# NVIDIA-Merlin/distributed-embeddings

Hardware: AMD Instinct MI355X
Metric: samples/sec (whole node) DLRM-Criteo-1TB bs/gpu=65536 (higher is better)
Workload: dtype bf16; 1 GPU; model=DLRM-Criteo-1TB, global_batch=65536, batch_per_gpu=65536, embedding_dim=128, parallelism=hybrid dp+mp (strategy=memory_balanced) x1

## Files before the change

distributed_embeddings_amd/csrc/bindings.cpp:

```cpp

#include <torch/extension.h>

#include <c10/hip/HIPStream.h>

#include "ops_api.h"

namespace {

#define CHECK_CUDA(x) TORCH_CHECK((x).is_cuda(), #x " must be on GPU")
#define CHECK_CONTIG(x) TORCH_CHECK((x).is_contiguous(), #x " must be contiguous")

inline hipStream_t current_stream() {
  return c10::hip::getCurrentHIPStream().stream();
}

int log2_ceil(int64_t v) {
  int b = 0;
  while ((int64_t(1) << b) < v) ++b;
  return b;
}


bool use_rocprim_sort() {
  static int v = -1;
// ... 479 lines not shown
              "rehash target must not be smaller");
  launch_hash_reinsert(old_keys.data_ptr<int64_t>(),
                       old_values.data_ptr<int64_t>(), old_keys.numel(),
                       new_keys.data_ptr<int64_t>(),
                       new_values.data_ptr<int64_t>(), new_keys.numel(),
                       current_stream());
}

static bool check_adagrad_state(const torch::Tensor& state,
                                const torch::Tensor& weight) {
  CHECK_CUDA(state); CHECK_CONTIG(state);
  const bool rowwise = state.dim() == 1 && state.size(0) == weight.size(0);
  TORCH_CHECK(rowwise || state.sizes() == weight.sizes(),
              "adagrad state shape mismatch: expected [vocab, width] "
              "(element-wise) or [vocab] (row-wise), got ", state.sizes(),
              " for weight ", weight.sizes());
  TORCH_CHECK(state.dtype() == torch::kFloat32, "adagrad state must be fp32");
  return rowwise;
}

static int64_t* sr_ptr(const std::optional<torch::Tensor>& sr,
                       const torch::Tensor& weight) {
  if (!sr.has_value()) return nullptr;
  const torch::Tensor& t = *sr;
  CHECK_CUDA(t); CHECK_CONTIG(t);
  TORCH_CHECK(t.dtype() == torch::kInt64 && t.dim() == 1 && t.numel() == 2,
              "sr must be an int64 [2] tensor {seed, step}");
  TORCH_CHECK(t.device() == weight.device(),
              "sr must be on the weight's device");
  TORCH_CHECK(weight.dtype() == torch::kBFloat16,
              "stochastic rounding needs a bf16 weight: an fp32 weight has "
              "nothing to round");
  return t.data_ptr<int64_t>();
}

static void check_adam_state(const torch::Tensor& state,
                             const torch::Tensor& weight, double beta1,
                             double beta2) {
  CHECK_CUDA(state); CHECK_CONTIG(state);
  TORCH_CHECK(state.dtype() == torch::kFloat32, "adam state must be fp32");
  TORCH_CHECK(state.dim() == 3 && state.size(0) == 2 &&
              state.size(1) == weight.size(0) &&
              state.size(2) == weight.size(1),
              "adam state shape mismatch: expected [2, vocab, width], got ",
              state.sizes(), " for weight ", weight.sizes());
  TORCH_CHECK(state.device() == weight.device(),
              "adam state must be on the weight's device");
  TORCH_CHECK(beta1 >= 0.0 && beta1 < 1.0 && beta2 >= 0.0 && beta2 < 1.0,
              "adam betas must lie in [0, 1), got (", beta1, ", ", beta2, ")");
}

void sparse_row_update(torch::Tensor weight, torch::Tensor state,
                       torch::Tensor ids, torch::Tensor grad, double lr,
                       double eps, bool adagrad,
                       std::optional<torch::Tensor> sr, int64_t adam_step,
                       double beta1, double beta2) {
  CHECK_CUDA(weight); CHECK_CUDA(ids); CHECK_CUDA(grad);
  CHECK_CONTIG(weight); CHECK_CONTIG(ids); CHECK_CONTIG(grad);
  TORCH_CHECK(weight.dtype() == torch::kFloat32 ||
              weight.dtype() == torch::kBFloat16);
  TORCH_CHECK(grad.dtype() == torch::kFloat32);
  TORCH_CHECK(ids.dtype() == torch::kInt64);
  int64_t* sr_p = sr_ptr(sr, weight);
  TORCH_CHECK(adam_step >= 0, "adam_step must not be negative");
  const bool adam = adam_step > 0;
  TORCH_CHECK(!(adam && adagrad), "adam_step and adagrad exclude each other");
  if (adam) check_adam_state(state, weight, beta1, beta2);
  const int64_t n = ids.numel();
  if (n == 0) return;
  float* state_ptr = nullptr;
  bool rowwise = false;
  if (adagrad) {
    rowwise = check_adagrad_state(state, weight);
    state_ptr = state.data_ptr<float>();
  }
  AdamConfig cfg{beta1, beta2, weight.size(0), nullptr, nullptr};
  if (adam) {
    state_ptr = state.data_ptr<float>();
    const double t = (double)adam_step;
    lr = lr * std::sqrt(1.0 - std::pow(beta2, t)) / (1.0 - std::pow(beta1, t));
  }
  launch_sparse_row_update(weight.data_ptr(),
                           weight.dtype() == torch::kBFloat16, state_ptr,
                           ids.data_ptr<int64_t>(), grad.data_ptr<float>(), n,
                           (int)weight.size(1), (float)lr, (float)eps, adagrad,
                           rowwise, sr_p, adam ? &cfg : nullptr,
                           current_stream());
}

void csr_fused_optimizer_apply(torch::Tensor weight, torch::Tensor state,
                               torch::Tensor values, torch::Tensor row_splits,
                               torch::Tensor grad_out, torch::Tensor lr,
                               bool mean, bool adagrad, double eps,
                               std::optional<torch::Tensor> per_id_w,
                               std::optional<torch::Tensor> sr,
                               std::optional<torch::Tensor> adam_step,
                               double beta1, double beta2) {
  CHECK_CUDA(weight); CHECK_CUDA(values); CHECK_CUDA(row_splits);
  CHECK_CUDA(grad_out); CHECK_CUDA(lr);
  CHECK_CONTIG(weight); CHECK_CONTIG(values); CHECK_CONTIG(row_splits);
  CHECK_CONTIG(grad_out);
  TORCH_CHECK(weight.dtype() == torch::kFloat32 ||
              weight.dtype() == torch::kBFloat16);
  TORCH_CHECK((grad_out.dtype() == torch::kFloat32 ||
               grad_out.dtype() == torch::kBFloat16) &&
              lr.dtype() == torch::kFloat32);
  const float* user_w = per_id_w_ptr(per_id_w, values);
  int64_t* sr_p = sr_ptr(sr, weight);
  const bool wbf16 = weight.dtype() == torch::kBFloat16;
  const int64_t num_rows = row_splits.numel() - 1;
  const int64_t nnz = values.numel();
  const int64_t vocab = weight.size(0);
  const int width = (int)weight.size(1);
  const bool adam = adam_step.has_value();
  if (adam) {
    TORCH_CHECK(!adagrad, "adam_step and adagrad exclude each other");
    check_adam_state(state, weight, beta1, beta2);
    const torch::Tensor& t = *adam_step;
    CHECK_CUDA(t); CHECK_CONTIG(t);
    TORCH_CHECK(t.dtype() == torch::kInt64 && t.dim() == 1 && t.numel() == 1,
                "adam_step must be an int64 [1] tensor");
    TORCH_CHECK(t.device() == weight.device(),
                "adam_step must be on the weight's device");
  }
  if (num_rows <= 0 || nnz <= 0) return;
  auto stream = current_stream();
  auto i64 = values.options();
  auto i32 = values.options().dtype(torch::kInt32);
  auto f32 = grad_out.options().dtype(torch::kFloat32);

  auto ss = build_sorted_segments(values, row_splits, vocab, mean, user_w,
                                  stream);
  launch_pad_seg_offsets(ss.seg.data_ptr<int64_t>(), nnz,
                         ss.num_unique.data_ptr<int32_t>(),
                         ss.bounds.data_ptr<int64_t>(), stream);
  auto long_rows = torch::empty({nnz}, i64);
  auto long_count = torch::empty({1}, i32);
  auto work_items = torch::empty({nnz / 64 + 64}, i64);
  auto n_work = torch::empty({1}, i32);
  float* state_ptr = nullptr;
  torch::Tensor scratch;
  float* scratch_ptr = nullptr;
  int64_t scratch_rows = 0;
  bool rowwise = false;
  if (adagrad) {
    rowwise = check_adagrad_state(state, weight);
    state_ptr = state.data_ptr<float>();
  }
  AdamConfig cfg{beta1, beta2, vocab, nullptr, nullptr};
  torch::Tensor a_t;
  if (adam) {
    state_ptr = state.data_ptr<float>();
    a_t = torch::empty({1}, f32);
    cfg.step = adam_step->data_ptr<int64_t>();
    cfg.a_t = a_t.data_ptr<float>();
  }
  if (adagrad || adam || wbf16) {
    scratch_rows = nnz / (128 + 1) + 1;
    scratch = torch::empty({scratch_rows, (int64_t)width}, f32);
    scratch_ptr = scratch.data_ptr<float>();
  }
  launch_sorted_optimizer_update(weight.data_ptr(), wbf16, state_ptr,
                                 (float)eps, ss.sorted_ids.data_ptr<int64_t>(),
                                 ss.seg.data_ptr<int64_t>(),
                                 ss.srow.data_ptr<int64_t>(), ss.sw_ptr(),
                                 grad_out.data_ptr(),
                                 grad_out.dtype() == torch::kBFloat16,
                                 lr.data_ptr<float>(),
                                 ss.num_unique.data_ptr<int32_t>(), nnz, width,
                                 long_rows.data_ptr<int64_t>(),
                                 long_count.data_ptr<int32_t>(),
                                 work_items.data_ptr<int64_t>(),
                                 n_work.data_ptr<int32_t>(), scratch_ptr,
                                 scratch_rows, adagrad, rowwise, sr_p,
                                 adam ? &cfg : nullptr, stream);
}

torch::Tensor stochastic_round_bf16(torch::Tensor x, int64_t seed,
                                    int64_t step, int64_t base_offset) {
  CHECK_CUDA(x); CHECK_CONTIG(x);
  TORCH_CHECK(x.dtype() == torch::kFloat32, "x must be fp32");
  TORCH_CHECK(base_offset >= 0, "base_offset must not be negative");
  auto out = torch::empty(x.sizes(), x.options().dtype(torch::kBFloat16));
  launch_stochastic_round_bf16(x.data_ptr<float>(), out.data_ptr(), x.numel(),
                               seed, step, base_offset, current_stream());
  return out;
}

torch::Tensor dot_interact_fwd(torch::Tensor feats, int64_t out_w) {
  CHECK_CUDA(feats); CHECK_CONTIG(feats);
  TORCH_CHECK(feats.dtype() == torch::kBFloat16, "feats must be bf16");
  TORCH_CHECK(feats.dim() == 3, "feats must be [B, F, D]");
  const int64_t B = feats.size(0);
  const int F = (int)feats.size(1), D = (int)feats.size(2);
  TORCH_CHECK(F <= 32 && D % 32 == 0, "F<=32 and D%32==0 required");
  const int tri_n = F * (F - 1) / 2;
  TORCH_CHECK(out_w >= tri_n + D, "out width too small");
  auto out = torch::empty({B, out_w}, feats.options());
  launch_dot_interact_fwd(feats.data_ptr(), out.data_ptr(), B, F, D,
                          (int)out_w, tri_n, current_stream());
  return out;
}

torch::Tensor dot_interact_fwd_packed(torch::Tensor bottom,
                                      torch::Tensor packed, torch::Tensor perm,
                                      int64_t out_w, bool sample_major) {
  CHECK_CUDA(bottom); CHECK_CUDA(packed); CHECK_CUDA(perm);
  CHECK_CONTIG(bottom); CHECK_CONTIG(packed); CHECK_CONTIG(perm);
  TORCH_CHECK(bottom.dtype() == torch::kBFloat16 &&
              packed.dtype() == torch::kBFloat16, "bf16 required");
  TORCH_CHECK(perm.dtype() == torch::kInt32, "perm must be int32");
  TORCH_CHECK(bottom.dim() == 2 && packed.dim() == 3, "bottom [B,D], packed 3-D");
  const int64_t B = bottom.size(0);
  const int D = (int)bottom.size(1);
  const int P = (int)(sample_major ? packed.size(1) : packed.size(0));
  TORCH_CHECK(packed.size(sample_major ? 0 : 1) == B && packed.size(2) == D,
              "shape mismatch");
  TORCH_CHECK(perm.numel() == P, "perm must have P entries");
  const int F = P + 1;
  TORCH_CHECK(F <= 32 && D % 32 == 0, "F<=32 and D%32==0 required");
  const int tri_n = F * (F - 1) / 2;
  TORCH_CHECK(out_w >= tri_n + D, "out width too small");
  const int64_t sb = sample_major ? P : 1;
  const int64_t sp = sample_major ? 1 : B;
  auto out = torch::empty({B, out_w}, bottom.options());
  launch_dot_interact_fwd_packed(bottom.data_ptr(), packed.data_ptr(),
                                 perm.data_ptr<int>(), out.data_ptr(), B, F, D,
                                 (int)out_w, tri_n, sb, sp, current_stream());
  return out;
}

std::vector<torch::Tensor> dot_interact_bwd_packed(torch::Tensor gout,
                                                   torch::Tensor bottom,
                                                   torch::Tensor packed,
                                                   torch::Tensor perm,
                                                   bool sample_major) {
  CHECK_CUDA(gout); CHECK_CUDA(bottom); CHECK_CUDA(packed); CHECK_CUDA(perm);
  CHECK_CONTIG(gout); CHECK_CONTIG(bottom); CHECK_CONTIG(packed);
  CHECK_CONTIG(perm);
  TORCH_CHECK(gout.dtype() == torch::kBFloat16 &&
              bottom.dtype() == torch::kBFloat16 &&
              packed.dtype() == torch::kBFloat16, "bf16 required");
  TORCH_CHECK(perm.dtype() == torch::kInt32, "perm must be int32");
  const int64_t B = bottom.size(0);
  const int D = (int)bottom.size(1);
  const int P = (int)(sample_major ? packed.size(1) : packed.size(0));
  TORCH_CHECK(perm.numel() == P, "perm must have P entries");
  TORCH_CHECK(packed.size(sample_major ? 0 : 1) == B && packed.size(2) == D,
              "shape mismatch");
  const int F = P + 1;
  const int tri_n = F * (F - 1) / 2;
  const int64_t sb = sample_major ? P : 1;
  const int64_t sp = sample_major ? 1 : B;
  auto gbottom = torch::empty_like(bottom);
  auto gpacked = torch::empty_like(packed);
  launch_dot_interact_bwd_packed(gout.data_ptr(), bottom.data_ptr(),
                                 packed.data_ptr(), perm.data_ptr<int>(),
                                 gbottom.data_ptr(), gpacked.data_ptr(), B, F,
                                 D, (int)gout.size(1), tri_n, sb, sp,
                                 current_stream());
  return {gbottom, gpacked};
}

torch::Tensor dot_interact_bwd(torch::Tensor gout, torch::Tensor feats) {
  CHECK_CUDA(gout); CHECK_CUDA(feats);
  CHECK_CONTIG(gout); CHECK_CONTIG(feats);
  TORCH_CHECK(gout.dtype() == torch::kBFloat16 &&
              feats.dtype() == torch::kBFloat16);
  const int64_t B = feats.size(0);
  const int F = (int)feats.size(1), D = (int)feats.size(2);
  const int tri_n = F * (F - 1) / 2;
  auto gfeats = torch::empty_like(feats);
  launch_dot_interact_bwd(gout.data_ptr(), feats.data_ptr(),
                          gfeats.data_ptr(), B, F, D, (int)gout.size(1), tri_n,
                          current_stream());
  return gfeats;
}

std::vector<torch::Tensor> relu_bwd_bias_grad(torch::Tensor grad_out,
                                              torch::Tensor y) {
  CHECK_CUDA(grad_out); CHECK_CUDA(y);
  CHECK_CONTIG(grad_out); CHECK_CONTIG(y);
  TORCH_CHECK(grad_out.dtype() == torch::kBFloat16 &&
              y.dtype() == torch::kBFloat16, "bf16 required");
  TORCH_CHECK(grad_out.dim() == 2 && grad_out.sizes() == y.sizes(),
              "grad_out and y must be [B, N]");
  const int64_t B = grad_out.size(0);
  const int64_t N = grad_out.size(1);
  TORCH_CHECK(N % 8 == 0 && N < (int64_t(1) << 31), "N % 8 == 0 required");
  auto grad_in = torch::empty_like(grad_out);
  if (B == 0 || N == 0) {
    return {grad_in, torch::zeros({N}, grad_out.options())};
  }
  auto bias_grad = torch::empty({N}, grad_out.options());
  int64_t rows_per_chunk = 0, num_chunks = 0;
  relu_bwd_bias_grad_plan(B, (int)N, &rows_per_chunk, &num_chunks);
  auto slab = torch::empty({num_chunks, N},
                           grad_out.options().dtype(torch::kFloat32));
  launch_relu_bwd_bias_grad(grad_out.data_ptr(), y.data_ptr(),
                            grad_in.data_ptr(), slab.data_ptr<float>(),
                            bias_grad.data_ptr(), B, (int)N, rows_per_chunk,
                            num_chunks, current_stream());
  return {grad_in, bias_grad};
}

}

PYBIND11_MODULE(TORCH_EXTENSION_NAME, m) {
  m.def("csr_lookup_forward", &csr_lookup_forward,
        "CSR segmented gather-reduce forward (gfx950)",
        pybind11::arg("params"), pybind11::arg("values"),
        pybind11::arg("row_splits"), pybind11::arg("mean"),
        pybind11::arg("out_bf16") = false,
        pybind11::arg("per_id_w") = pybind11::none());
  m.def("csr_lookup_forward_q8", &csr_lookup_forward_q8,
        "CSR gather-reduce from an int8 row-wise quantized table (gfx950)",
        pybind11::arg("packed"), pybind11::arg("values"),
        pybind11::arg("row_splits"), pybind11::arg("mean"),
        pybind11::arg("out_bf16") = false,
        pybind11::arg("per_id_w") = pybind11::none());
  m.def("quantize_rows_q8", &quantize_rows_q8,
        "fp32/bf16 [n, width] -> int8 row-wise packed [n, width + 8] (gfx950)",
        pybind11::arg("weight"));
  m.def("dequantize_rows_q8", &dequantize_rows_q8,
        "int8 row-wise packed [n, width + 8] -> fp32 [n, width] (gfx950)",
        pybind11::arg("packed"));
  m.def("csr_lookup_backward", &csr_lookup_backward,
        "sparse backward: sort + unique + segmented sum (gfx950)",
        pybind11::arg("grad_out"), pybind11::arg("values"),
        pybind11::arg("row_splits"), pybind11::arg("vocab"),
        pybind11::arg("mean"), pybind11::arg("per_id_w") = pybind11::none());
  m.def("csr_lookup_weight_grad", &csr_lookup_weight_grad,
        "gradient of the per-id weights of a weighted lookup (gfx950)",
        pybind11::arg("grad_out"), pybind11::arg("params"),
        pybind11::arg("values"), pybind11::arg("row_splits"),
        pybind11::arg("mean"));
  m.def("debug_sort_ids", &debug_sort_ids,
        "TESTS ONLY: the backward's id sort -> (sorted_ids, sorted_pos)",
        pybind11::arg("values"), pybind11::arg("vocab"),
        pybind11::arg("variant") = -1, pybind11::arg("sort") = "default");
  m.def("debug_sorted_segments", &debug_sorted_segments,
        "TESTS ONLY: the backward's sorted-segment view -> (sorted_ids, "
        "srow, sw or None, seg, unique_ids, num_unique, bounds)",
        pybind11::arg("values"), pybind11::arg("row_splits"),
        pybind11::arg("vocab"), pybind11::arg("mean"),
        pybind11::arg("per_id_w") = pybind11::none(),
        pybind11::arg("padded") = false, pybind11::arg("variant") = -1,
        pybind11::arg("sort") = "default");
  m.def("debug_sort_variant_tiles", &debug_sort_variant_tiles,
        "TESTS ONLY: keys per block of each radix-sort tile variant");
  m.def("row_to_split", &row_to_split, "COO rows -> CSR splits (gfx950)");
  m.def("hash_rehash", &hash_rehash,
        "re-insert occupied (key,value) pairs into a larger hash (gfx950)");
  m.def("integer_lookup", &integer_lookup,
        "open-addressing hash vocab build + lookup (gfx950)");
  m.def("sparse_row_update", &sparse_row_update,
        "fused sparse SGD/Adagrad/row-wise Adagrad/lazy Adam row update "
        "(gfx950)",
        pybind11::arg("weight"), pybind11::arg("state"), pybind11::arg("ids"),
        pybind11::arg("grad"), pybind11::arg("lr"), pybind11::arg("eps"),
        pybind11::arg("adagrad"), pybind11::arg("sr") = pybind11::none(),
        pybind11::arg("adam_step") = 0, pybind11::arg("beta1") = 0.9,
        pybind11::arg("beta2") = 0.999);
  m.def("csr_fused_optimizer_apply", &csr_fused_optimizer_apply,
        "in-backward fused SGD/Adagrad/row-wise Adagrad/lazy Adam update "
        "(gfx950)",
        pybind11::arg("weight"), pybind11::arg("state"),
        pybind11::arg("values"), pybind11::arg("row_splits"),
        pybind11::arg("grad_out"), pybind11::arg("lr"), pybind11::arg("mean"),
        pybind11::arg("adagrad"), pybind11::arg("eps"),
        pybind11::arg("per_id_w") = pybind11::none(),
        pybind11::arg("sr") = pybind11::none(),
        pybind11::arg("adam_step") = pybind11::none(),
        pybind11::arg("beta1") = 0.9, pybind11::arg("beta2") = 0.999);
  m.def("stochastic_round_bf16", &stochastic_round_bf16,
        "fp32 -> bf16 with the fused optimizers' stochastic rounding (gfx950)",
        pybind11::arg("x"), pybind11::arg("seed"), pybind11::arg("step") = 0,
        pybind11::arg("base_offset") = 0);
  m.def("dot_interact_fwd_packed", &dot_interact_fwd_packed,
        "pairwise-dot interaction on (bottom, packed, perm) (MFMA, gfx950)");
  m.def("dot_interact_bwd_packed", &dot_interact_bwd_packed,
        "packed interaction backward -> (gbottom, gpacked) (MFMA, gfx950)");
  m.def("dot_interact_fwd", &dot_interact_fwd,
        "fused DLRM pairwise-dot interaction forward (MFMA bf16, gfx950)");
  m.def("dot_interact_bwd", &dot_interact_bwd,
        "fused DLRM pairwise-dot interaction backward (MFMA bf16, gfx950)");
  m.def("relu_bwd_bias_grad", &relu_bwd_bias_grad,
        "ReLU backward + bias gradient in one pass -> (grad_in, bias_grad) "
        "(gfx950)");
}
```

distributed_embeddings_amd/csrc/ops_api.h:

```cpp
#pragma once

#include <hip/hip_runtime.h>

#include <cstddef>
#include <cstdint>

void launch_csr_lookup_forward(const void* params, bool params_bf16,
                               const int64_t* values, const int64_t* splits,
                               const float* per_id_w, void* out, bool out_bf16,
                               int64_t num_rows, int64_t nnz, int64_t vocab,
                               int width, bool mean, int64_t* long_rows,
                               int32_t* long_count, int64_t* work_items,
                               int32_t* n_work, hipStream_t stream);

void launch_csr_lookup_forward_q8(const void* packed, const int64_t* values,
                                  const int64_t* splits, const float* per_id_w,
                                  void* out, bool out_bf16, int64_t num_rows,
                                  int64_t nnz, int64_t vocab, int width,
                                  bool mean, int64_t* long_rows,
                                  int32_t* long_count, int64_t* work_items,
                                  int32_t* n_work, hipStream_t stream);
void launch_quantize_rows_q8(const void* in, bool in_bf16, void* packed,
                             int64_t n, int width, hipStream_t stream);
void launch_dequantize_rows_q8(const void* packed, float* out, int64_t n,
                               int width, hipStream_t stream);

void launch_row_to_split(const int64_t* rows, int64_t nnz, int64_t num_rows,
                         int64_t* splits, hipStream_t stream);

size_t csr_backward_temp_bytes(int64_t nnz);

void launch_expand_row_ids(const int64_t* splits, int64_t num_rows,
                           int64_t nnz, int32_t* row_ids, float* w, bool mean,
                           const float* user_w, hipStream_t stream);

void launch_csr_weight_grad(const void* params, bool params_bf16,
                            const void* grad_out, bool grad_bf16,
                            const int64_t* values, const int32_t* row_ids,
                            const int64_t* splits, bool mean, float* dw,
                            int64_t nnz, int64_t vocab, int width,
                            hipStream_t stream);

hipError_t run_inclusive_scan_i32(void* temp, size_t temp_bytes,
                                  const int32_t* in, int32_t* out, int64_t n,
                                  hipStream_t stream);

void launch_mark_heads(const int64_t* sorted_ids, int64_t n, int64_t vocab,
                       int32_t* head, hipStream_t stream);

void launch_scatter_unique(const int64_t* sorted_ids, const int32_t* head,
                           const int32_t* pos, int64_t n, int64_t* unique_ids,
                           int64_t* seg_offsets, int32_t* num_unique,
                           hipStream_t stream);

void launch_gather_sorted(const int32_t* perm, const int32_t* row_ids,
                          const float* w, int64_t n, int64_t* srow, float* sw,
                          hipStream_t stream);

void launch_find_valid_bounds(const int64_t* sorted_ids, int64_t n,
                              int64_t vocab, int64_t* valid_end,
                              hipStream_t stream);

void launch_set_seg_end(int64_t* seg_offsets, const int32_t* num_unique,
                        const int64_t* valid_end, hipStream_t stream);

void launch_integer_lookup(const int64_t* keys, int64_t n, int64_t* tkeys,
                           int64_t* tvals, int64_t capacity, int32_t* counts,
                           int64_t max_tokens, void* temp, size_t temp_bytes,
                           int32_t* scratch_flags, int32_t* scratch_pos,
                           int64_t* avail, int32_t* navail, int32_t* next_avail,
                           int64_t* out, hipStream_t stream);

size_t integer_lookup_temp_bytes(int64_t max_tokens);

void launch_hash_reinsert(const int64_t* old_keys, const int64_t* old_vals,
                          int64_t old_cap, int64_t* tkeys, int64_t* tvals,
                          int64_t capacity, hipStream_t stream);

void launch_pad_seg_offsets(int64_t* seg, int64_t n, const int32_t* num_unique,
                            const int64_t* valid_end, hipStream_t stream);

struct AdamConfig {
  double b1, b2;
  int64_t vocab;
  int64_t* step;
  float* a_t;
};

void launch_sorted_optimizer_update(void* weight, bool weight_bf16,
                                    float* state, float eps,
                                    const int64_t* sorted_ids,
                                    const int64_t* seg, const int64_t* srow,
                                    const float* sw, const void* grad_out,
                                    bool grad_bf16,
                                    const float* lr, const int32_t* nu_ptr,
                                    int64_t max_segs, int width,
                                    int64_t* long_rows, int32_t* long_count,
                                    int64_t* work_items, int32_t* n_work,
                                    float* long_scratch, int64_t scratch_rows,
                                    bool adagrad, bool rowwise, int64_t* sr,
                                    const AdamConfig* adam,
                                    hipStream_t stream);

void launch_sparse_row_update(void* weight, bool weight_bf16, float* state,
                              const int64_t* ids, const float* grad,
                              int64_t num_rows, int width, float lr, float eps,
                              bool adagrad, bool rowwise, int64_t* sr,
                              const AdamConfig* adam, hipStream_t stream);

void launch_stochastic_round_bf16(const float* x, void* out, int64_t n,
                                  int64_t seed, int64_t step,
                                  int64_t base_offset, hipStream_t stream);

void launch_dot_interact_fwd_packed(const void* bottom, const void* packed,
                                    const int* perm, void* out, int64_t B,
                                    int F, int D, int out_w, int tri_n,
                                    int64_t sb, int64_t sp,
                                    hipStream_t stream);
void launch_dot_interact_bwd_packed(const void* gout, const void* bottom,
                                    const void* packed, const int* perm,
                                    void* gbottom, void* gpacked, int64_t B,
                                    int F, int D, int out_w, int tri_n,
                                    int64_t sb, int64_t sp,
                                    hipStream_t stream);
void launch_dot_interact_fwd(const void* feats, void* out, int64_t B, int F,
                             int D, int out_w, int tri_n, hipStream_t stream);
void launch_dot_interact_bwd(const void* gout, const void* feats, void* gfeats,
                             int64_t B, int F, int D, int out_w, int tri_n,
                             hipStream_t stream);

void relu_bwd_bias_grad_plan(int64_t B, int N, int64_t* rows_per_chunk,
                             int64_t* num_chunks);
void launch_relu_bwd_bias_grad(const void* grad_out, const void* y,
                               void* grad_in, float* slab, void* bias_grad,
                               int64_t B, int N, int64_t rows_per_chunk,
                               int64_t num_chunks, hipStream_t stream);

size_t custom_radix_sort_hist_elems(int64_t n);
int custom_radix_sort_num_variants();
int custom_radix_sort_variant_tile(int variant);

void custom_radix_sort_keys(const uint64_t* keys_in, uint64_t* keys_out,
                            uint64_t* keys_tmp, int32_t* hist,
                            int32_t* scan_sums, int64_t n, int begin_bit,
                            int end_bit, int variant, hipStream_t stream);

void launch_mask_oob_pack(const int64_t* ids, int64_t n, int64_t vocab,
                          uint64_t* packed, hipStream_t stream);
void launch_unpack_sorted(const uint64_t* packed, int64_t n,
                          int64_t* sorted_ids, int32_t* sorted_pos,
                          hipStream_t stream);
hipError_t run_sort_keys_u64(void* temp, size_t temp_bytes,
                             const uint64_t* keys_in, uint64_t* keys_out,
                             int64_t n, int begin_bit, int end_bit,
                             hipStream_t stream);
size_t rocprim_sort_keys_temp_bytes(int64_t n);
```

distributed_embeddings_amd/ops/mlp.py:

```python

import os
from typing import Tuple

import torch
from torch import nn

from . import _backend


def relu_bwd_bias_grad(grad_out: torch.Tensor,
                       y: torch.Tensor) -> Tuple[torch.Tensor, torch.Tensor]:
    if (grad_out.is_cuda and grad_out.dim() == 2
            and grad_out.dtype == torch.bfloat16 and y.dtype == torch.bfloat16
            and grad_out.shape == y.shape and grad_out.shape[1] % 8 == 0
            and grad_out.is_contiguous() and y.is_contiguous()):
        g, gb = _backend.ops().relu_bwd_bias_grad(grad_out, y)
        return g, gb
    g = torch.ops.aten.threshold_backward(grad_out, y, 0)
    return g, g.sum(0)


class _LinearReLU(torch.autograd.Function):

    @staticmethod
    def forward(ctx, x, w, b):
        xb = x.to(torch.bfloat16)
        wb = w.to(torch.bfloat16)
        y = torch.addmm(b.to(torch.bfloat16), xb, wb.t())
        torch.relu_(y)
        ctx.save_for_backward(xb, wb, y)
        ctx.x_dtype = x.dtype
        return y

    @staticmethod
    @torch.autograd.function.once_differentiable
    def backward(ctx, grad_out):
        xb, wb, y = ctx.saved_tensors
        g, gb = relu_bwd_bias_grad(grad_out, y)
        gx = None
        if ctx.needs_input_grad[0]:
            gx = g.mm(wb).to(ctx.x_dtype)
        gw = g.t().mm(xb)
        return gx, gw, gb


class MLP(nn.Sequential):

    def _fused(self, x: torch.Tensor) -> bool:
        return (x.is_cuda and x.dim() == 2 and torch.is_autocast_enabled()
                and torch.get_autocast_dtype("cuda") == torch.bfloat16
                and os.environ.get("DE_FUSED_MLP", "1") != "0"
                and _backend.available())

    def forward(self, input):
        if not self._fused(input):
            return super().forward(input)
        mods = list(self)
        h = input
        i = 0
        while i < len(mods):
            m = mods[i]
            if (isinstance(m, nn.Linear) and m.bias is not None
                    and m.weight.dtype == torch.float32
                    and m.bias.dtype == torch.float32
                    and i + 1 < len(mods) and isinstance(mods[i + 1], nn.ReLU)
                    and h.dim() == 2):
                h = _LinearReLU.apply(h, m.weight, m.bias)
                i += 2
            else:
                h = m(h)
                i += 1
        return h
```

setup.py:

```python

import os

from setuptools import setup

os.environ.setdefault("PYTORCH_ROCM_ARCH", "gfx950")

from torch.utils.cpp_extension import BuildExtension, CUDAExtension

ext = CUDAExtension(
    name="distributed_embeddings_amd._hip_ops",
    sources=[
        "distributed_embeddings_amd/csrc/bindings.cpp",
        "distributed_embeddings_amd/csrc/embedding_ops.hip",
        "distributed_embeddings_amd/csrc/dot_interact.hip",
        "distributed_embeddings_amd/csrc/radix_sort.hip",
        "distributed_embeddings_amd/csrc/mlp_ops.hip",
    ],
    extra_compile_args={
        "cxx": ["-O3", "-std=c++17"],
        "nvcc": ["-O3", "-std=c++17"],
    },
)

setup(
    name="distributed_embeddings_amd",
    version="0.1.0",
    packages=[
        "distributed_embeddings_amd",
        "distributed_embeddings_amd.ops",
        "distributed_embeddings_amd.layers",
        "distributed_embeddings_amd.parallel",
        "distributed_embeddings_amd.models",
        "distributed_embeddings_amd.utils",
    ],
    ext_modules=[ext],
    cmdclass={"build_ext": BuildExtension},
)
```

Measured before the change: 17.86 million samples/s.

## Add split-K MFMA kernel for MLP weight gradients with tall-skinny shapes

Adds a custom split-K bf16 MFMA GEMM for the linear weight gradient g^T x, where K is the large batch dimension (65536) and M, N are small layer widths. Each workgroup accumulates a K-slice into an fp32 slab, and a second kernel reduces the slices and rounds to bf16. The goal is to fill the GPU on shapes where a standard GEMM yields few output tiles. The cost is an extra fp32 slab write and read, a second launch, and a host-side plan call on every backward.

```diff
diff --git a/distributed_embeddings_amd/csrc/bindings.cpp b/distributed_embeddings_amd/csrc/bindings.cpp
--- a/distributed_embeddings_amd/csrc/bindings.cpp
+++ b/distributed_embeddings_amd/csrc/bindings.cpp
@@ -805,6 +805,40 @@
                             bias_grad.data_ptr(), B, (int)N, rows_per_chunk,
                             num_chunks, current_stream());
   return {grad_in, bias_grad};
+}
+
+torch::Tensor wgrad_splitk(torch::Tensor g, torch::Tensor x, int64_t splitk,
+                           int64_t tile) {
+  CHECK_CUDA(g); CHECK_CUDA(x);
+  CHECK_CONTIG(g); CHECK_CONTIG(x);
+  TORCH_CHECK(g.dtype() == torch::kBFloat16 && x.dtype() == torch::kBFloat16,
+              "bf16 required");
+  TORCH_CHECK(g.dim() == 2 && x.dim() == 2 && g.size(0) == x.size(0),
+              "g must be [K, M] and x [K, N]");
+  const int64_t K = g.size(0), M = g.size(1), N = x.size(1);
+  TORCH_CHECK(splitk >= 0, "splitk must not be negative");
+  TORCH_CHECK(tile >= -1 && tile <= 2, "tile must be -1 (plan), 0, 1 or 2");
+  WgradSplitkPlan plan;
+  TORCH_CHECK(wgrad_splitk_plan_with(K, M, N, splitk, (int)tile, &plan),
+              "wgrad_splitk takes K >= 1, M % 8 == 0 and N % 8 == 0 or "
+              "N <= 16 (tile 2 for N <= 16 only); got K=", K, " M=", M,
+              " N=", N, " tile=", tile);
+  TORCH_CHECK(reinterpret_cast<uintptr_t>(g.data_ptr()) % 16 == 0 &&
+              reinterpret_cast<uintptr_t>(x.data_ptr()) % 16 == 0,
+              "operands must be 16-byte aligned");
+  auto gw = torch::empty({M, N}, g.options());
+  auto slab = torch::empty({plan.splitk, M, plan.np},
+                           g.options().dtype(torch::kFloat32));
+  launch_wgrad_splitk(g.data_ptr(), x.data_ptr(), slab.data_ptr<float>(),
+                      gw.data_ptr(), K, (int)M, (int)N, plan,
+                      current_stream());
+  return gw;
+}
+
+std::vector<int64_t> wgrad_splitk_plan_py(int64_t K, int64_t M, int64_t N) {
+  WgradSplitkPlan plan;
+  if (!wgrad_splitk_plan(K, M, N, &plan)) return {0, 0, -1};
+  return {plan.use ? 1 : 0, plan.splitk, plan.cfg};
 }
 
 }
@@ -891,4 +925,10 @@
   m.def("relu_bwd_bias_grad", &relu_bwd_bias_grad,
         "ReLU backward + bias gradient in one pass -> (grad_in, bias_grad) "
         "(gfx950)");
-}
+  m.def("wgrad_splitk", &wgrad_splitk,
+        "Linear weight gradient bf16(g^T x), split-K (MFMA bf16, gfx950)",
+        pybind11::arg("g"), pybind11::arg("x"), pybind11::arg("splitk") = 0,
+        pybind11::arg("tile") = -1);
+  m.def("wgrad_splitk_plan", &wgrad_splitk_plan_py,
+        "(use, splitk, tile geometry) for g [K, M], x [K, N]");
+}
diff --git a/distributed_embeddings_amd/csrc/ops_api.h b/distributed_embeddings_amd/csrc/ops_api.h
--- a/distributed_embeddings_amd/csrc/ops_api.h
+++ b/distributed_embeddings_amd/csrc/ops_api.h
@@ -136,6 +136,20 @@
                                int64_t B, int N, int64_t rows_per_chunk,
                                int64_t num_chunks, hipStream_t stream);
 
+struct WgradSplitkPlan {
+  int cfg;
+  int splitk;
+  int64_t kslice;
+  int np;
+  bool use;
+};
+bool wgrad_splitk_plan(int64_t K, int64_t M, int64_t N, WgradSplitkPlan* plan);
+bool wgrad_splitk_plan_with(int64_t K, int64_t M, int64_t N, int64_t splitk,
+                            int tile, WgradSplitkPlan* plan);
+void launch_wgrad_splitk(const void* g, const void* x, float* slab, void* gw,
+                         int64_t K, int M, int N, const WgradSplitkPlan& plan,
+                         hipStream_t stream);
+
 size_t custom_radix_sort_hist_elems(int64_t n);
 int custom_radix_sort_num_variants();
 int custom_radix_sort_variant_tile(int variant);
diff --git a/distributed_embeddings_amd/csrc/wgrad_splitk.hip b/distributed_embeddings_amd/csrc/wgrad_splitk.hip
--- /dev/null
+++ b/distributed_embeddings_amd/csrc/wgrad_splitk.hip
@@ -0,0 +1,300 @@
+
+#include <hip/hip_runtime.h>
+
+#include "ops_api.h"
+
+namespace {
+
+constexpr int THREADS = 256;
+
+typedef __attribute__((ext_vector_type(8))) short bf16x8;
+typedef __attribute__((ext_vector_type(4))) float f32x4;
+typedef short v4i16_t __attribute__((vector_size(8)));
+typedef __attribute__((address_space(3))) v4i16_t lds_v4i16_t;
+
+__device__ __forceinline__ unsigned short f32_to_bf16_rne(float f) {
+  unsigned int u = __float_as_uint(f);
+  if (f != f) return 0x7FC0;
+  u += 0x7FFFu + ((u >> 16) & 1u);
+  return (unsigned short)(u >> 16);
+}
+
+template <int W>
+__device__ __forceinline__ int swz(int row, int col) {
+  const int sw = (((row & 3) << 2) | ((row >> 2) & 3)) & (W / 8 - 1);
+  return row * W + ((((col >> 3) ^ sw) << 3) | (col & 7));
+}
+
+template <int W, int BK, bool NARROW>
+struct Stage {
+  static constexpr int C = W / 8;
+  static constexpr int TOTAL = BK * C;
+  static constexpr int NL = (TOTAL + THREADS - 1) / THREADS;
+  bf16x8 v[NL];
+
+  __device__ __forceinline__ void load(const short* __restrict__ src,
+                                       int64_t k0, int64_t kend, int col0,
+                                       int ld) {
+#pragma unroll
+    for (int it = 0; it < NL; ++it) {
+      const int chunk = it * THREADS + threadIdx.x;
+      const int64_t k = k0 + chunk / C;
+      const int col = col0 + (chunk % C) * 8;
+      const bf16x8 z = {0, 0, 0, 0, 0, 0, 0, 0};
+      v[it] = z;
+      if (chunk < TOTAL && k < kend) {
+        if (!NARROW) {
+          if (col < ld) {
+            v[it] = *reinterpret_cast<const bf16x8*>(src + k * ld + col);
+          }
+        } else {
+#pragma unroll
+          for (int j = 0; j < 8; ++j) {
+            if (col + j < ld) v[it][j] = src[k * ld + col + j];
+          }
+        }
+      }
+    }
+  }
+
+  __device__ __forceinline__ void store(short* img) const {
+#pragma unroll
+    for (int it = 0; it < NL; ++it) {
+      const int chunk = it * THREADS + threadIdx.x;
+      if (chunk < TOTAL) {
+        *reinterpret_cast<bf16x8*>(&img[swz<W>(chunk / C, (chunk % C) * 8)]) =
+            v[it];
+      }
+    }
+  }
+};
+
+template <int W>
+__device__ __forceinline__ bf16x8 tr_fragment(const short* img, int r0, int c0,
+                                              int lane) {
+  const int row = r0 + (lane >> 4) * 8 + ((lane & 15) >> 2);
+  const int col = c0 + (lane & 3) * 4;
+  const v4i16_t lo = __builtin_amdgcn_ds_read_tr16_b64_v4i16(
+      (lds_v4i16_t*)(img + swz<W>(row, col)));
+  const v4i16_t hi = __builtin_amdgcn_ds_read_tr16_b64_v4i16(
+      (lds_v4i16_t*)(img + swz<W>(row + 4, col)));
+  return bf16x8{lo[0], lo[1], lo[2], lo[3], hi[0], hi[1], hi[2], hi[3]};
+}
+
+template <int WAVES_M, int WAVES_N, int WM, int WN, int BK, bool NARROW_X>
+__global__ __launch_bounds__(THREADS) void wgrad_splitk_partial(
+    const short* __restrict__ g, const short* __restrict__ x,
+    float* __restrict__ slab, int64_t K, int M, int N, int Np, int64_t kslice,
+    int tiles_n) {
+  static_assert(WAVES_M * WAVES_N * 64 == THREADS, "4 waves");
+  static_assert(BK % 32 == 0, "whole MFMA k-steps");
+  constexpr int BM = WAVES_M * WM * 16;
+  constexpr int BN = WAVES_N * WN * 16;
+  constexpr int BUF = BK * (BM + BN);
+  extern __shared__ short lds[];
+
+  const int lane = threadIdx.x & 63;
+  const int wave = __builtin_amdgcn_readfirstlane(threadIdx.x >> 6);
+  const int wm0 = (wave / WAVES_N) * WM * 16;
+  const int wn0 = (wave % WAVES_N) * WN * 16;
+  const int m0 = (blockIdx.x / tiles_n) * BM;
+  const int n0 = (blockIdx.x % tiles_n) * BN;
+  const int64_t kbeg = (int64_t)blockIdx.y * kslice;
+  int64_t kend = kbeg + kslice;
+  if (kend > K) kend = K;
+  const int nsteps = (int)((kend - kbeg + BK - 1) / BK);
+
+  f32x4 acc[WN][WM];
+#pragma unroll
+  for (int j = 0; j < WN; ++j) {
+#pragma unroll
+    for (int i = 0; i < WM; ++i) acc[j][i] = f32x4{0.f, 0.f, 0.f, 0.f};
+  }
+
+  Stage<BM, BK, false> sg;
+  Stage<BN, BK, NARROW_X> sx;
+  sg.load(g, kbeg, kend, m0, M);
+  sx.load(x, kbeg, kend, n0, N);
+  sg.store(lds);
+  sx.store(lds + BK * BM);
+  __syncthreads();
+
+  for (int s = 0; s < nsteps; ++s) {
+    const short* gimg = lds + (s & 1) * BUF;
+    const short* ximg = gimg + BK * BM;
+    const bool more = s + 1 < nsteps;
+    if (more) {
+      sg.load(g, kbeg + (int64_t)(s + 1) * BK, kend, m0, M);
+      sx.load(x, kbeg + (int64_t)(s + 1) * BK, kend, n0, N);
+    }
+#pragma unroll
+    for (int kk = 0; kk < BK; kk += 32) {
+      bf16x8 a[WM], b[WN];
+#pragma unroll
+      for (int i = 0; i < WM; ++i) {
+        a[i] = tr_fragment<BM>(gimg, kk, wm0 + i * 16, lane);
+      }
+#pragma unroll
+      for (int j = 0; j < WN; ++j) {
+        b[j] = tr_fragment<BN>(ximg, kk, wn0 + j * 16, lane);
+      }
+#pragma unroll
+      for (int j = 0; j < WN; ++j) {
+#pragma unroll
+        for (int i = 0; i < WM; ++i) {
+          acc[j][i] = __builtin_amdgcn_mfma_f32_16x16x32_bf16(b[j], a[i],
+                                                              acc[j][i], 0, 0, 0);
+        }
+      }
+    }
+    if (more) {
+      short* nxt = lds + ((s + 1) & 1) * BUF;
+      sg.store(nxt);
+      sx.store(nxt + BK * BM);
+    }
+    __syncthreads();
+  }
+
+  float* out = slab + (int64_t)blockIdx.y * M * Np;
+#pragma unroll
+  for (int i = 0; i < WM; ++i) {
+    const int m = m0 + wm0 + i * 16 + (lane & 15);
+#pragma unroll
+    for (int j = 0; j < WN; ++j) {
+      const int n = n0 + wn0 + j * 16 + 4 * (lane >> 4);
+      if (m < M && n < Np) {
+        *reinterpret_cast<f32x4*>(&out[(int64_t)m * Np + n]) = acc[j][i];
+      }
+    }
+  }
+}
+
+constexpr int FIN_QUADS = 64;
+constexpr int FIN_LANES = 4;
+
+__global__ __launch_bounds__(FIN_QUADS* FIN_LANES) void wgrad_splitk_finish(
+    const float* __restrict__ slab, unsigned short* __restrict__ gw, int S,
+    int M, int N, int Np) {
+  __shared__ f32x4 part[FIN_LANES][FIN_QUADS];
+  const int q = threadIdx.x % FIN_QUADS;
+  const int l = threadIdx.x / FIN_QUADS;
+  const int64_t total = (int64_t)M * (Np / 4);
+  const int64_t quad = (int64_t)blockIdx.x * FIN_QUADS + q;
+  const int64_t stride = (int64_t)M * Np;
+  f32x4 s = {0.f, 0.f, 0.f, 0.f};
+  if (quad < total) {
+#pragma unroll 4
+    for (int r = l; r < S; r += FIN_LANES) {
+      s += *reinterpret_cast<const f32x4*>(&slab[r * stride + quad * 4]);
+    }
+  }
+  part[l][q] = s;
+  __syncthreads();
+  if (l == 0 && quad < total) {
+    f32x4 t = part[0][q];
+#pragma unroll
+    for (int i = 1; i < FIN_LANES; ++i) t += part[i][q];
+    const int64_t m = quad / (Np / 4);
+    const int n = (int)(quad % (Np / 4)) * 4;
+    unsigned short* dst = gw + m * N + n;
+    if (N == Np) {
+      typedef __attribute__((ext_vector_type(4))) unsigned short u16x4;
+      const u16x4 o = {f32_to_bf16_rne(t[0]), f32_to_bf16_rne(t[1]),
+                       f32_to_bf16_rne(t[2]), f32_to_bf16_rne(t[3])};
+      *reinterpret_cast<u16x4*>(dst) = o;
+    } else {
+#pragma unroll
+      for (int j = 0; j < 4; ++j) {
+        if (n + j < N) dst[j] = f32_to_bf16_rne(t[j]);
+      }
+    }
+  }
+}
+
+constexpr int BK_ALL = 64;
+constexpr int CFG_BM[3] = {128, 64, 128};
+constexpr int CFG_BN[3] = {128, 64, 16};
+
+template <int WAVES_M, int WAVES_N, int WM, int WN, bool NARROW_X>
+void launch_partial(const void* g, const void* x, float* slab, int64_t K,
+                    int M, int N, int Np, int64_t kslice, int splitk,
+                    hipStream_t stream) {
+  constexpr int BM = WAVES_M * WM * 16, BN = WAVES_N * WN * 16;
+  const int tiles_m = (M + BM - 1) / BM, tiles_n = (N + BN - 1) / BN;
+  const size_t lds = (size_t)2 * BK_ALL * (BM + BN) * sizeof(short);
+  hipLaunchKernelGGL(
+      (wgrad_splitk_partial<WAVES_M, WAVES_N, WM, WN, BK_ALL, NARROW_X>),
+      dim3(tiles_m * tiles_n, splitk), dim3(THREADS), lds, stream,
+      (const short*)g, (const short*)x, slab, K, M, N, Np, kslice, tiles_n);
+}
+
+}
+
+bool wgrad_splitk_plan(int64_t K, int64_t M, int64_t N, WgradSplitkPlan* plan) {
+  return wgrad_splitk_plan_with(K, M, N, 0, -1, plan);
+}
+
+bool wgrad_splitk_plan_with(int64_t K, int64_t M, int64_t N, int64_t splitk,
+                            int tile, WgradSplitkPlan* plan) {
+  if (K < 1 || M < 8 || M % 8 != 0 || N < 1 || M >= (1 << 24) ||
+      N >= (1 << 24) || (N % 8 != 0 && N > 16)) {
+    return false;
+  }
+  int cfg;
+  if (N <= 16) {
+    cfg = 2;
+  } else if (M <= 64 || N <= 64) {
+    cfg = 1;
+  } else {
+    cfg = 0;
+  }
+  if (tile >= 0) {
+    if (tile > 2 || (tile == 2) != (N <= 16)) return false;
+    cfg = tile;
+  }
+  const int64_t np = (N + 3) / 4 * 4;
+  const int64_t tiles = ((M + CFG_BM[cfg] - 1) / CFG_BM[cfg]) *
+                        ((N + CFG_BN[cfg] - 1) / CFG_BN[cfg]);
+  int64_t sk = 512 / tiles;
+  const int64_t max_sk = (K + BK_ALL - 1) / BK_ALL;
+  if (sk > max_sk) sk = max_sk;
+  if (sk < 1) sk = 1;
+  const int64_t operand_bytes = K * (M + N) * 2;
+  while (sk > 1 && 2 * sk * M * np * 4 > operand_bytes) sk /= 2;
+  if (splitk > 0) sk = splitk < max_sk ? splitk : max_sk;
+  int64_t kslice = (K + sk - 1) / sk;
+  kslice = (kslice + BK_ALL - 1) / BK_ALL * BK_ALL;
+  sk = (K + kslice - 1) / kslice;
+  if (sk > 65535) return false;
+  plan->cfg = cfg;
+  plan->splitk = (int)sk;
+  plan->kslice = kslice;
+  plan->np = (int)np;
+  plan->use = K >= 4096 && sk >= 8;
+  return true;
+}
+
+void launch_wgrad_splitk(const void* g, const void* x, float* slab, void* gw,
+                         int64_t K, int M, int N, const WgradSplitkPlan& plan,
+                         hipStream_t stream) {
+  const int np = plan.np;
+  if (plan.cfg == 0) {
+    launch_partial<2, 2, 4, 4, false>(g, x, slab, K, M, N, np, plan.kslice,
+                                      plan.splitk, stream);
+  } else if (plan.cfg == 1) {
+    launch_partial<2, 2, 2, 2, false>(g, x, slab, K, M, N, np, plan.kslice,
+                                      plan.splitk, stream);
+  } else if (N % 8 == 0) {
+    launch_partial<4, 1, 2, 1, false>(g, x, slab, K, M, N, np, plan.kslice,
+                                      plan.splitk, stream);
+  } else {
+    launch_partial<4, 1, 2, 1, true>(g, x, slab, K, M, N, np, plan.kslice,
+                                     plan.splitk, stream);
+  }
+  const int64_t quads = (int64_t)M * (np / 4);
+  hipLaunchKernelGGL(wgrad_splitk_finish,
+                     dim3((unsigned)((quads + FIN_QUADS - 1) / FIN_QUADS)),
+                     dim3(FIN_QUADS * FIN_LANES), 0, stream,
+                     (const float*)slab, (unsigned short*)gw, plan.splitk, M,
+                     N, np);
+}
diff --git a/distributed_embeddings_amd/ops/mlp.py b/distributed_embeddings_amd/ops/mlp.py
--- a/distributed_embeddings_amd/ops/mlp.py
+++ b/distributed_embeddings_amd/ops/mlp.py
@@ -20,6 +20,21 @@
     return g, g.sum(0)
 
 
+def _wgrad_routed(k: int, m: int, n: int) -> bool:
+    return bool(_backend.ops().wgrad_splitk_plan(k, m, n)[0])
+
+
+def weight_grad(g: torch.Tensor, xb: torch.Tensor) -> torch.Tensor:
+    if (g.is_cuda and g.dim() == 2 and xb.dim() == 2
+            and g.dtype == torch.bfloat16 and xb.dtype == torch.bfloat16
+            and g.is_contiguous() and xb.is_contiguous()
+            and g.data_ptr() % 16 == 0 and xb.data_ptr() % 16 == 0
+            and os.environ.get("DE_WGRAD_SPLITK", "1") != "0"
+            and _wgrad_routed(g.shape[0], g.shape[1], xb.shape[1])):
+        return _backend.ops().wgrad_splitk(g, xb)
+    return g.t().mm(xb)
+
+
 class _LinearReLU(torch.autograd.Function):
 
     @staticmethod
@@ -40,7 +55,7 @@
         gx = None
         if ctx.needs_input_grad[0]:
             gx = g.mm(wb).to(ctx.x_dtype)
-        gw = g.t().mm(xb)
+        gw = weight_grad(g, xb)
         return gx, gw, gb
 
 
diff --git a/setup.py b/setup.py
--- a/setup.py
+++ b/setup.py
@@ -15,6 +15,7 @@
         "distributed_embeddings_amd/csrc/dot_interact.hip",
         "distributed_embeddings_amd/csrc/radix_sort.hip",
         "distributed_embeddings_amd/csrc/mlp_ops.hip",
+        "distributed_embeddings_amd/csrc/wgrad_splitk.hip",
     ],
     extra_compile_args={
         "cxx": ["-O3", "-std=c++17"],
```

Result: faster. 20.24 million samples/s, median of 6 (+13.3%).
